# TorchIO-project/torchio

Measured on AMD Instinct MI355X. Metric: volumes/s (256^3 float32) for Compose[affine+elastic+bias+blur+noise], higher is better.
Workload: dtype f32; 1 GPU; Compose[Affine(+-10deg,0.9-1.1,+-5mm),ElasticDeformation(7^3cp,7.5mm),BiasField,Blur(0.5-2mm),Noise] on 1x256^3 f32, per-instance params; batch_per_gpu=8, global_batch=8, noise_rng=philox, resample_precision=tight, stencil_precision=fast, parallelism=batch-split x1 (no data-path collective)

## Files before the change

### include/tio_hip.h

```cpp
#ifndef TIO_HIP_H
#define TIO_HIP_H

#include <stdint.h>

#ifdef __cplusplus
extern "C" {
#endif

#define TIO_ABI_VERSION 18
#define TIO_MAX_IMAGES 8

typedef enum tio_status {
  TIO_OK = 0,
  TIO_ERR_INVALID_ARGUMENT = -1,
  TIO_ERR_UNSUPPORTED_DTYPE = -2,
  TIO_ERR_LAUNCH = -3,
  TIO_ERR_NO_DEVICE = -4,
  TIO_ERR_UNSUPPORTED_CONFIG = -5
} tio_status;

typedef enum tio_dtype {
  TIO_F32 = 0,
  TIO_F64 = 1,
  TIO_F16 = 2,
// ... 276 lines not shown

int tio_kspace_add_spikes(const void* x, void* y, int32_t dtype, int32_t batch, int32_t channels, const int32_t shape[3],
                          const int32_t* params_dev, int32_t params_words, int32_t max_count, const float* tables_dev,
                          const float* peaks_dev, const uint8_t* active_dev, void* stream);

#define TIO_MAX_SEGMENTS 32

int tio_kspace_segment_mix(const void* const* segments, int32_t n_segments, const int32_t* bounds,
                           const float* mix_dev, void* out, int32_t dtype, int32_t batch,
                           int32_t channels, const int32_t shape[3], const uint8_t* active_dev,
                           void* stream);
int tio_kspace_mix_table(int32_t length, int32_t n_segments, const int32_t* bounds, float* table_host);

#define TIO_HOST_MT_STATE_BYTES 2688
typedef struct tio_host_mt_state { uint64_t opaque[TIO_HOST_MT_STATE_BYTES / 8]; } tio_host_mt_state;
int tio_host_mt19937_seed(tio_host_mt_state* state, uint64_t seed);
int tio_host_mt19937_randn(tio_host_mt_state* state, float* out, int64_t n, int32_t n_threads);

int64_t tio_host_mt19937_plan_words(int64_t n);
int tio_host_mt19937_plan(tio_host_mt_state* state, int64_t n, uint32_t* plan_host, int64_t capacity_words, int64_t* used_words,
                          int32_t n_threads);
int64_t tio_host_mt19937_plan_begin(tio_host_mt_state* state, int64_t n, uint32_t* plan_host, int64_t capacity_words, int32_t n_threads);
int tio_host_mt19937_plan_end(int64_t handle, int64_t* used_words);
int tio_mt19937_randn_device(const uint32_t* plan_host, const uint32_t* plan_dev, float* out_dev, void* stream);
int tio_host_mt19937_plan_prefix(tio_host_mt_state* state, int64_t n, uint32_t* plan_host, int64_t capacity_words, int64_t* prefix_words,
                                 int64_t* used_words, int64_t* total_blocks);
int tio_host_mt19937_segment_polynomials(int64_t segment_blocks, int32_t count, uint32_t* out);
int tio_mt19937_device_snapshots(uint32_t* plan_dev, int64_t total_blocks, int64_t segment_blocks, const uint32_t* polys_dev, void* stream);
int tio_mt19937_add_noise_device(const uint32_t* plan_host, const uint32_t* plan_dev, const float* x_dev, float* out_dev,
                                 int64_t n_per_element, float mean, float std, const float* mean_dev, const float* std_dev,
                                 void* stream);

#define TIO_PCA_MAX_CHANNELS 1024

int64_t tio_channel_scatter_workspace_bytes(int32_t batch, int32_t channels, int64_t voxels);
int tio_channel_scatter_plan(int32_t batch, int32_t channels, int64_t voxels, int32_t out[4]);
int tio_channel_scatter(const float* x, int32_t batch, int32_t channels, int64_t voxels, double* mean, double* scatter,
                        void* workspace_dev, int64_t workspace_bytes, void* stream);

int tio_channel_project(const float* x, int32_t batch, int32_t channels, int64_t voxels, const float* center_dev,
                        const float* weights_dev, const float* offset_dev, int32_t components, int32_t clip, float* y,
                        void* stream);

#define TIO_POINTS_BLOCK_DOUBLES 40
#define TIO_POINTS_MAX_ITERATIONS 50
#define TIO_POINTS_TOLERANCE 1.0e-7
int tio_points_warp(const float* points, float* out, int8_t* status, int64_t n_total, const int32_t* offsets_host,
                    const int32_t* offsets_dev, int32_t batch, const double* blocks_dev, const float* control_points_dev,
                    int64_t control_floats, void* stream);

#define TIO_CENTRE_SEGMENT 2048
#define TIO_CENTRE_MAX_LABELS 64
typedef struct tio_centre_record {
  double total;
  int32_t invalid;
  int32_t reserved;
} tio_centre_record;
int tio_centre_law_sums(const void* weights, int32_t element_type, int32_t label_mode, const double* label_values,
                        const float* label_weights, int32_t n_labels, const int32_t shape[3], const int32_t patch[3],
                        double* prefix_dev, tio_centre_record* record_dev, void* stream);
int tio_centre_draw(const void* weights, int32_t element_type, int32_t label_mode, const double* label_values,
                    const float* label_weights, int32_t n_labels, const int32_t shape[3], const int32_t patch[3],
                    const double* prefix_dev, const tio_centre_record* record_dev, int64_t n_draws, uint64_t seed,
                    const double* uniforms_dev, double* uniforms_out_dev, int64_t* centres_dev, int32_t* corners_dev, void* stream);

int tio_patch_gather(const void* x, void* y, int32_t element_bytes, int32_t channels, const int32_t shape[3], const int32_t patch[3],
                     const int32_t* corners_dev, int32_t n_patches, void* stream);

typedef struct tio_nifti_layout {
  int32_t disk_type;
  int32_t swap_bytes;
  int32_t shape[3];
  int32_t channels;
  int32_t scaled;
  double slope, inter;
} tio_nifti_layout;
int tio_nifti_decode(const void* raw_dev, void* y, int32_t out_type, int32_t batch, const tio_nifti_layout* layout, void* stream);

int tio_abi_version(void);
const char* tio_last_error(void);
int tio_device_count(void);
void tio_reload_env(void);
int tio_launch_streams(int64_t bytes_written);

#ifdef __cplusplus
}
#endif
#endif
```

### torchio_amd/csrc/api.hip

```cpp
#include <stdarg.h>
#include <stdio.h>
#include <stdlib.h>
#include <string.h>

#include <algorithm>
#include <atomic>
#include <mutex>

#include "common.hpp"

namespace tio {

static thread_local char g_error[512] = "";

void set_error(const char* fmt, ...) {
  va_list ap;
  va_start(ap, fmt);
  vsnprintf(g_error, sizeof(g_error), fmt, ap);
  va_end(ap);
}

int fail(int status, const char* fmt, ...) {
  va_list ap;
  va_start(ap, fmt);
  vsnprintf(g_error, sizeof(g_error), fmt, ap);
  va_end(ap);
  return status;
}

int check_launch(const char* what) {
  const hipError_t err = hipGetLastError();
  if (err != hipSuccess) return fail(TIO_ERR_LAUNCH, "%s: launch failed: %s", what, hipGetErrorString(err));
  return TIO_OK;
}

static std::atomic<const EnvSwitches*> g_env{nullptr};
static std::mutex g_env_mu;

static const EnvSwitches* parse_env() {
  EnvSwitches* e = new EnvSwitches();
  auto num = [](const char* name, int unset) { const char* v = getenv(name); return v != nullptr ? atoi(v) : unset; };
  e->nearest_kernel = num("TIO_NEAREST_KERNEL", 1) != 0;
  if (const char* v = getenv("TIO_NEAREST_EPS")) { e->has_nearest_eps = 1; e->nearest_eps = static_cast<float>(atof(v)); }
  if (const char* v = getenv("TIO_RESAMPLE_PATH")) e->resample_path = strcmp(v, "gather") == 0 ? 1 : (strcmp(v, "tile") == 0 ? 2 : 0);
  e->tile_ablate = num("TIO_TILE_ABLATE", 0);
  e->resample_exact = getenv("TIO_RESAMPLE_EXACT") != nullptr;
  if (const char* v = getenv("TIO_FAST_KERNEL")) e->fast_kernel = strcmp(v, "brick") == 0 ? 1 : (strcmp(v, "planned") == 0 ? 2 : 0);
  e->planned_lean = num("TIO_PLANNED_LEAN", 1) != 0;
  e->exact_plan = num("TIO_EXACT_PLAN", -1);
  e->exact_lean = num("TIO_EXACT_LEAN", -1);
  e->lean_interleave = num("TIO_LEAN_INTERLEAVE", 1);
  e->lean_multi = num("TIO_LEAN_MULTI", 1);
  e->nearest_exact = num("TIO_NEAREST_EXACT", 1);
  e->lean_pair = num("TIO_LEAN_PAIR", 1);
  e->lean_label = num("TIO_LEAN_LABEL", 1);
  e->fast_fill_recheck = num("TIO_FAST_FILL_RECHECK", 1) != 0;
  e->conv_no_fuse = getenv("TIO_CONV_NO_FUSE") != nullptr;
  e->conv_ring = getenv("TIO_CONV_RING") != nullptr;
  if (const char* v = getenv("TIO_STREAM_BYTES")) e->stream_bytes = std::max<long long>(0, atoll(v));
  return e;
}

const EnvSwitches& env_switches() {
  const EnvSwitches* e = g_env.load(std::memory_order_acquire);
  if (e != nullptr) return *e;
  std::lock_guard<std::mutex> lock(g_env_mu);
  e = g_env.load(std::memory_order_acquire);
  if (e == nullptr) { e = parse_env(); g_env.store(e, std::memory_order_release); }
  return *e;
}

}

extern "C" void tio_reload_env(void) {
  std::lock_guard<std::mutex> lock(tio::g_env_mu);
  tio::g_env.store(tio::parse_env(), std::memory_order_release);
}

extern "C" int tio_launch_streams(int64_t bytes_written) { return tio::launch_streams(bytes_written) ? 1 : 0; }

extern "C" int tio_abi_version(void) { return TIO_ABI_VERSION; }

extern "C" const char* tio_last_error(void) { return tio::g_error; }

extern "C" int tio_device_count(void) {
  int n = 0;
  if (hipGetDeviceCount(&n) != hipSuccess) {
    (void)hipGetLastError();
    return 0;
  }
  return n;
}
```

### torchio_amd/csrc/common.hpp

```cpp
#pragma once

#include <hip/hip_runtime.h>
#include <stdint.h>

#include <type_traits>

#include "../../include/tio_hip.h"

namespace tio {

void set_error(const char* fmt, ...);
int fail(int status, const char* fmt, ...);
int check_launch(const char* what);

struct EnvSwitches {
  int nearest_kernel = 1;
  int has_nearest_eps = 0;
  float nearest_eps = 0.0f;
  int resample_path = 0;
  int tile_ablate = 0;
  int resample_exact = 0;
  int fast_kernel = 0;
  int planned_lean = 1;
  int exact_plan = -1;
  int exact_lean = -1;
  int nearest_exact = 1;
  int lean_pair = 1;
  int lean_label = 1;
  int lean_multi = 1;
  int lean_interleave = 1;
  int fast_fill_recheck = 1;
  int conv_no_fuse = 0;
  int conv_ring = 0;
  int64_t stream_bytes = -1;
};
const EnvSwitches& env_switches();

constexpr int64_t kStreamBytes = 256ll << 20;
inline bool launch_streams(int64_t bytes_written) {
  const int64_t threshold = env_switches().stream_bytes;
  return bytes_written > (threshold >= 0 ? threshold : kStreamBytes);
}

__device__ __forceinline__ float bf16_bits_to_float(uint16_t h) {
  return __uint_as_float(static_cast<uint32_t>(h) << 16);
}

__device__ __forceinline__ uint16_t float_to_bf16_bits(float f) {
  uint32_t x = __float_as_uint(f);
  if ((x & 0x7FFFFFFFu) > 0x7F800000u) return 0x7FC0u;
  x += 0x7FFFu + ((x >> 16) & 1u);
  return static_cast<uint16_t>(x >> 16);
}

template <int DT>
struct Elem;
template <>
struct Elem<TIO_F32> {
  using type = float;
  static __device__ __forceinline__ float load(const void* p, int64_t i) { return static_cast<const float*>(p)[i]; }
  static __device__ __forceinline__ void store(void* p, int64_t i, float v) { static_cast<float*>(p)[i] = v; }
};
template <>
struct Elem<TIO_F64> {
  using type = double;
  static __device__ __forceinline__ float load(const void* p, int64_t i) {
    return static_cast<float>(static_cast<const double*>(p)[i]);
  }
  static __device__ __forceinline__ void store(void* p, int64_t i, float v) {
    static_cast<double*>(p)[i] = static_cast<double>(v);
  }
};
template <>
struct Elem<TIO_F16> {
  using type = _Float16;
  static __device__ __forceinline__ float load(const void* p, int64_t i) {
    return static_cast<float>(static_cast<const _Float16*>(p)[i]);
  }
  static __device__ __forceinline__ void store(void* p, int64_t i, float v) {
    asm volatile("" : "+v"(v));
    static_cast<_Float16*>(p)[i] = static_cast<_Float16>(v);
  }
};
template <>
struct Elem<TIO_BF16> {
  using type = uint16_t;
  static __device__ __forceinline__ float load(const void* p, int64_t i) {
    return bf16_bits_to_float(static_cast<const uint16_t*>(p)[i]);
  }
  static __device__ __forceinline__ void store(void* p, int64_t i, float v) {
    static_cast<uint16_t*>(p)[i] = float_to_bf16_bits(v);
  }
};
#define TIO_INT_ELEM(CODE, T)                                                                  \
  template <>                                                                                  \
  struct Elem<CODE> {                                                                          \
    using type = T;                                                                            \
    static __device__ __forceinline__ float load(const void* p, int64_t i) {                   \
      return static_cast<float>(static_cast<const T*>(p)[i]);                                  \
    }                                                                                          \
    static __device__ __forceinline__ void store(void* p, int64_t i, float v) {                \
      static_cast<T*>(p)[i] = static_cast<T>(static_cast<int64_t>(v));     \
    }                                                                                          \
  };
TIO_INT_ELEM(TIO_U8, uint8_t)
TIO_INT_ELEM(TIO_I8, int8_t)
TIO_INT_ELEM(TIO_I16, int16_t)
TIO_INT_ELEM(TIO_I32, int32_t)
TIO_INT_ELEM(TIO_I64, int64_t)
#undef TIO_INT_ELEM

__device__ __forceinline__ float load_as_float(const void* p, int dtype, int64_t i) {
  switch (dtype) {
    case TIO_F32: return Elem<TIO_F32>::load(p, i);
    case TIO_F64: return Elem<TIO_F64>::load(p, i);
    case TIO_F16: return Elem<TIO_F16>::load(p, i);
// ... 154 lines not shown
```

### torchio_amd/csrc/resample.hip

```cpp
#include <type_traits>
#include <stdlib.h>
#include <string.h>

#include <mutex>
#include <vector>
#include <algorithm>

#include "resample_args.hpp"
#include "resample_coords.hpp"

namespace tio {

constexpr int kTileI = 8;
constexpr int kRowsPerBlock = 4;
constexpr int kLanes = 64;
constexpr int kMaxCpLds = 6144;
constexpr int kLdsFloatsPerCU = 40960;
constexpr int kPlannedMinBricks = 12288;
constexpr int kTileMinCap = 6144;
constexpr int kTileBlocksPerCU = 3;

template <int DT>
__device__ __forceinline__ void sample_interior(const ImgArgs& g, int b, int64_t n_in, int64_t n_out, int64_t o_idx,
                                                const float (&w)[8], int base, int dJK, int dK, int offn) {
// ... 425 lines not shown
#define TIO_CALL(DT) sample_boundary<DT>(g, b, n_in, n_out, o_idx, w, off, okbits, mask, offn, okn)
        TIO_DISPATCH_IMAGE(DTMODE, g.dtype, TIO_CALL)
#undef TIO_CALL
      }
    }
  }
}

}

#include "resample_exact_chain.hpp"
#include "resample_tile.hpp"
#include "resample_line.hpp"
#include "resample_plan.hpp"
#include "resample_fast.hpp"
#include "resample_lean_exact.hpp"
#include "resample_nearest.hpp"

namespace {
struct PlanSlot {
  int device;
  hipStream_t stream;
  int* ptr = nullptr;
  size_t cap = 0;
  std::mutex busy;
};
struct PlanLease {
  std::unique_lock<std::mutex> hold;
  int* ptr = nullptr;
};
}

static PlanLease plan_workspace(hipStream_t s, size_t bytes) {
  static std::mutex registry_mu;
  static std::vector<PlanSlot*> registry;
  PlanLease lease;
  int device = 0;
  if (hipGetDevice(&device) != hipSuccess) return lease;
  PlanSlot* slot = nullptr;
  {
    std::lock_guard<std::mutex> lock(registry_mu);
    for (PlanSlot* sl : registry)
      if (sl->device == device && sl->stream == s) slot = sl;
    if (slot == nullptr) {
      slot = new PlanSlot();
      slot->device = device; slot->stream = s;
      registry.push_back(slot);
    }
  }
  lease.hold = std::unique_lock<std::mutex>(slot->busy);
  if (slot->cap < bytes) {
    if (slot->ptr != nullptr) {
      (void)hipStreamSynchronize(s);
      (void)hipFree(slot->ptr);
      slot->ptr = nullptr; slot->cap = 0;
    }
    if (hipMalloc(&slot->ptr, bytes) != hipSuccess) { slot->ptr = nullptr; return lease; }
    if (hipMemsetAsync(slot->ptr, 0, tio::kPlanHeaderInts * sizeof(int), s) != hipSuccess) { (void)hipFree(slot->ptr); slot->ptr = nullptr; return lease; }
    slot->cap = bytes;
  }
  lease.ptr = slot->ptr;
  return lease;
}

namespace {
using namespace tio;

using RowsKernel = void (*)(ResampleArgs);
using BrickKernel = void (*)(ResampleArgs, const int*);
using LeanKernel = void (*)(LeanArgs);

unsigned magic_u32(unsigned n) { return n > 1 ? 0xFFFFFFFFu / n + 1u : 0u; }

template <typename Args>
int set_tiles(Args& a, int ti, int tj, int tk, unsigned* blocks) {
  a.tiles_k = (a.Ko + tk - 1) / tk; a.tiles_j = (a.Jo + tj - 1) / tj; a.tiles_i = (a.Io + ti - 1) / ti;
  a.magic_k = magic_u32(a.tiles_k); a.magic_j = magic_u32(a.tiles_j); a.magic_i = magic_u32(a.tiles_i);
  const int64_t n = static_cast<int64_t>(a.B) * a.tiles_i * a.tiles_j * a.tiles_k;
  if (n >= (1LL << 31)) return fail(TIO_ERR_INVALID_ARGUMENT, "tio_resample3d: grid too large");
  *blocks = static_cast<unsigned>(n);
  return TIO_OK;
}

template <typename Kernel>
int reserve_lds(Kernel kernel, size_t bytes) {
  if (bytes > 48 * 1024 && hipFuncSetAttribute(reinterpret_cast<const void*>(kernel), hipFuncAttributeMaxDynamicSharedMemorySize, static_cast<int>(bytes)) != hipSuccess)
    return fail(TIO_ERR_LAUNCH, "tio_resample3d: cannot reserve %zu bytes of LDS", bytes);
  return TIO_OK;
}

int control_floats(const ResampleArgs& a) { return a.cp != nullptr ? a.ni * a.nj * a.nk * 3 : 0; }
bool control_points_fit_lds(const ResampleArgs& a) { return control_floats(a) > 0 && control_floats(a) <= kMaxCpLds; }

struct Plan {
  PlanLease lease;
  int* ptr = nullptr;
  bool made_ahead = false;
};
int acquire_plan(const tio_resample_geom* geom, size_t need, hipStream_t s, Plan* plan) {
  if (geom->plan_dev != nullptr && geom->plan_bytes >= static_cast<int64_t>(need) && (reinterpret_cast<uintptr_t>(geom->plan_dev) & 15) == 0) {
    plan->ptr = static_cast<int*>(const_cast<void*>(geom->plan_dev)) + kPlanHeaderInts;
    plan->made_ahead = true;
    return TIO_OK;
  }
  plan->lease = plan_workspace(s, need);
  if (plan->lease.ptr == nullptr) return fail(TIO_ERR_LAUNCH, "tio_resample3d: cannot allocate the brick plan");
  plan->ptr = plan->lease.ptr + kPlanHeaderInts;
  return TIO_OK;
}

void enqueue_planner(const ResampleArgs& a, int* plan, int n_items, hipStream_t s) {
  const int plan_lanes = plan_group(a.cp != nullptr);
  const int plan_threads = n_items * plan_lanes > a.B ? n_items * plan_lanes : a.B;
  const dim3 plan_grid((plan_threads + 255) / 256);
  with_bools([&](auto elastic) { hipLaunchKernelGGL((plan_bricks_kernel<elastic.value, 16, 16, 16>), plan_grid, dim3(256), 0, s, a, plan, n_items); }, a.cp != nullptr);
}

int plan_bricks(const tio_resample_geom* geom, ResampleArgs& a, size_t plan_need, hipStream_t s, Plan* plan, int* n_items) {
  unsigned bricks = 0;
  if (const int st = set_tiles(a, 16, 16, 16, &bricks)) return st;
  *n_items = static_cast<int>(bricks);
  if (const int st = acquire_plan(geom, plan_need, s, plan)) return st;
  if (!plan->made_ahead) enqueue_planner(a, plan->ptr, *n_items, s);
  return TIO_OK;
}

struct FoldedMin {
  uint32_t* keys = nullptr;
  MinOuts outs{};
  int channels = 0;
};
int take_folded_min(ResampleArgs& a, bool allowed, hipStream_t s, FoldedMin* m) {
  for (int i = 0; i < a.n_images; i++) m->channels += a.img[i].out_min != nullptr ? a.img[i].channels : 0;
  if (m->channels == 0 || m->channels > kMinChannels || !allowed) {
    m->channels = 0;
    for (int i = 0; i < a.n_images; i++) a.img[i].out_min = nullptr;
    return TIO_OK;
  }
  int cap = 0;
  m->keys = min_workspace(s, m->channels * kMinSlots, &cap, 1);
  if (m->keys == nullptr) return fail(TIO_ERR_LAUNCH, "tio_resample3d: cannot allocate the reduction workspace");
  int slot = 0;
  for (int i = 0; i < a.n_images; i++)
    if (a.img[i].out_min != nullptr) {
      a.img[i].min_keys = m->keys + slot * kMinSlots;
      for (int c = 0; c < a.img[i].channels; c++) m->outs.p[slot + c] = a.img[i].out_min + c;
      slot += a.img[i].channels;
    }
  return TIO_OK;
}

void finish_folded_min(const FoldedMin& m, hipStream_t s) {
  if (m.channels > 0)
    hipLaunchKernelGGL(min_finish_kernel, dim3(static_cast<unsigned>(m.channels)), dim3(kMinSlots), 0, s, m.keys, m.outs, m.channels);
}

int check_geometry(const tio_resample_geom* geom, ResampleArgs& a) {
  if (geom->batch < 0) return fail(TIO_ERR_INVALID_ARGUMENT, "tio_resample3d: negative batch");
  if (geom->batch == 0) return TIO_OK;
  if (geom->mapping_dev == nullptr) return fail(TIO_ERR_INVALID_ARGUMENT, "tio_resample3d: mapping_dev is null");
  for (int d = 0; d < 3; d++) {
    if (geom->in_shape[d] < 1 || geom->out_shape[d] < 1)
      return fail(TIO_ERR_INVALID_ARGUMENT, "tio_resample3d: shapes must be >= 1");
  }
  const int64_t n_in = static_cast<int64_t>(geom->in_shape[0]) * geom->in_shape[1] * geom->in_shape[2];
  const int64_t n_out = static_cast<int64_t>(geom->out_shape[0]) * geom->out_shape[1] * geom->out_shape[2];
  if (n_in >= (1LL << 31) || n_out >= (1LL << 31))
    return fail(TIO_ERR_INVALID_ARGUMENT, "tio_resample3d: more than 2^31 voxels per channel");
  if (geom->passthrough_dev != nullptr && n_in != n_out)
    return fail(TIO_ERR_INVALID_ARGUMENT, "tio_resample3d: passthrough needs in_shape == out_shape");
  if (geom->control_points_dev != nullptr) {
    for (int d = 0; d < 3; d++)
      if (geom->cp_shape[d] < 1) return fail(TIO_ERR_INVALID_ARGUMENT, "tio_resample3d: bad cp_shape");
  }

  a.B = geom->batch;
  a.I = geom->in_shape[0]; a.J = geom->in_shape[1]; a.K = geom->in_shape[2];
  a.Io = geom->out_shape[0]; a.Jo = geom->out_shape[1]; a.Ko = geom->out_shape[2];
  a.affine_first = geom->affine_first;
  a.mapping = geom->mapping_dev;
  a.mapping_batched = geom->mapping_batched;
  a.cp = geom->control_points_dev;
  a.cp_batched = geom->cp_batched;
  a.ni = geom->cp_shape[0]; a.nj = geom->cp_shape[1]; a.nk = geom->cp_shape[2];
  a.cp_skip = geom->cp_skip_dev;
  a.passthrough = geom->passthrough_dev;
  const float* sp = geom->affine_first ? geom->in_spacing : geom->out_spacing;
  a.unit_spacing = 1;
  a.short_div = 1;
  for (int d = 0; d < 3; d++) {
    a.sp[d] = sp[d];
    a.rsp[d] = 1.0f / sp[d];
    if (sp[d] != 1.0f) a.unit_spacing = 0;
    const int size = geom->in_shape[d];
// ... 336 lines not shown
    if (const int st = reserve_lds(kernel_label_one, r.lds)) return st;
    la.lab_in = nn.img[0].in; la.lab_out = nn.img[0].out; la.lab_es = label->es;
  }
  int launches_left = channels;
  bool have_first = false;
  for (int i = 0; i < a.n_images; i++) {
    const ImgArgs& g = a.img[i];
    for (int c = 0; c < g.channels; c++) {
      --launches_left;
      if (pairs && !have_first && launches_left > 0) {
        set_lean_channel<false>(la, g, c);
        have_first = true;
        continue;
      }
      la.last_use = !plan.made_ahead && launches_left == 0;
      la.min_keys = (fold && g.min_keys != nullptr) ? g.min_keys + c * kMinSlots : nullptr;
      const bool with_label = label_here && launches_left == 0;
      if (have_first) set_lean_channel<true>(la, g, c);
      else set_lean_channel<false>(la, g, c);
      const LeanKernel launch = have_first ? (with_label ? kernel_label_pair : kernel_pair) : (with_label ? kernel_label_one : kernel);
      have_first = false;
      hipLaunchKernelGGL(launch, grid, block, r.lds, s, la);
      if (kernel_multi != nullptr) hipLaunchKernelGGL(kernel_multi, grid_multi, block, r.lds, s, la);
    }
  }
  finish_folded_min(fm, s);
  if (label_here) label->es = 0;
  return check_launch("tio_resample3d");
}

int resample3d_impl(const tio_resample_geom* geom, int32_t n_images, const tio_resample_image* images, void* stream, bool* folded) {
  *folded = false;
  if (geom == nullptr || images == nullptr) return fail(TIO_ERR_INVALID_ARGUMENT, "tio_resample3d: null argument");
  if (n_images < 1 || n_images > TIO_MAX_IMAGES)
    return fail(TIO_ERR_INVALID_ARGUMENT, "tio_resample3d: n_images=%d not in [1, %d]", n_images, TIO_MAX_IMAGES);
  ResampleArgs a{};
  int status = check_geometry(geom, a);
  if (status != TIO_OK || a.B == 0) return status;
  ResampleArgs pv = a, spl = a;
  pv.any_linear = 1;
  NearestArgs nn = make_nearest_args(a);
  FloatGroup group;
  const EnvSwitches& env = env_switches();
  if ((status = sort_images(n_images, images, env, a, pv, spl, nn, group)) != TIO_OK) return status;

  hipStream_t s = static_cast<hipStream_t>(stream);
  LabelRide label;
  if (nn.n_images > 0) {
    const bool floats_alone = a.n_images > 0 && pv.n_images == 0 && spl.n_images == 0 && !group.any_adjoint;
    if ((status = launch_nearest(nn, a.short_div != 0, floats_alone, env, s, &label)) != TIO_OK) return status;
    if (a.n_images == 0 && pv.n_images == 0 && spl.n_images == 0) return check_launch("tio_resample3d");
  }
  if (pv.n_images > 0) {
    if ((status = launch_label_pv(pv, s)) != TIO_OK) return status;
    if (a.n_images == 0 && spl.n_images == 0) return check_launch("tio_resample3d");
  }
  if (spl.n_images > 0) {
    if ((status = launch_bspline(spl, s)) != TIO_OK) return status;
    if (a.n_images == 0) return check_launch("tio_resample3d");
  }

  const FloatRoad road = choose_float_road(*geom, a, group, env);
  apply_road(a, road);
  switch (road.kind) {
    case kRoadGather: status = launch_gather(a, group.dtmode, s); break;
    case kRoadBrick: case kRoadPlannedBrick: case kRoadFastBrick: status = launch_brick(geom, a, road, group.dtmode, s); break;
    case kRoadPlannedFast: status = launch_planned_fast(geom, a, road, pv.n_images == 0, s, folded); break;
    case kRoadPlannedLean: case kRoadLeanExact: status = launch_lean(geom, a, road, pv.n_images == 0, nn, &label, s, folded); break;
  }
  if (label.es != 0) launch_nearest_exact(nn, label.es, label.blocks, label.lds, s);
  return status;
}

int choose_plan_road(const tio_resample_geom* geom, ResampleArgs* a, FloatRoad* road) {
  const int status = check_geometry(geom, *a);
  if (status != TIO_OK) return status;
  a->any_linear = 1;
  *road = choose_float_road(*geom, *a, FloatGroup{}, env_switches());
  return TIO_OK;
}

}

extern "C" int64_t tio_resample3d_plan_bytes(const tio_resample_geom* geom) {
  if (geom == nullptr || geom->batch < 1) return 0;
  ResampleArgs a{};
  FloatRoad road;
  return choose_plan_road(geom, &a, &road) == TIO_OK ? static_cast<int64_t>(road.plan_need) : 0;
}

extern "C" int tio_resample3d_plan(const tio_resample_geom* geom, void* plan_dev, int64_t plan_bytes, void* stream) {
  if (geom == nullptr || geom->batch < 1) return tio::fail(TIO_ERR_INVALID_ARGUMENT, "tio_resample3d_plan: no geometry / empty batch");
  ResampleArgs a{};
  FloatRoad road;
  if (const int st = choose_plan_road(geom, &a, &road)) return st;
  if (road.plan_need == 0) return tio::fail(TIO_ERR_INVALID_ARGUMENT, "tio_resample3d_plan: this geometry's launch does not start from a plan");
  if (plan_dev == nullptr || plan_bytes < static_cast<int64_t>(road.plan_need) || (reinterpret_cast<uintptr_t>(plan_dev) & 15) != 0)
    return tio::fail(TIO_ERR_INVALID_ARGUMENT, "tio_resample3d_plan: the plan needs %zu bytes, 16-byte aligned", road.plan_need);
  apply_road(a, road);
  unsigned bricks = 0;
  if (const int st = set_tiles(a, 16, 16, 16, &bricks)) return st;
  hipStream_t s = static_cast<hipStream_t>(stream);
  if (a.plan_multi && hipMemsetAsync(plan_dev, 0, kPlanHeaderInts * sizeof(int), s) != hipSuccess)
    return tio::fail(TIO_ERR_LAUNCH, "tio_resample3d_plan: cannot reset the brick plan");
  enqueue_planner(a, static_cast<int*>(plan_dev) + kPlanHeaderInts, static_cast<int>(bricks), s);
  return tio::check_launch("tio_resample3d_plan");
}

extern "C" int tio_resample3d(const tio_resample_geom* geom, int32_t n_images, const tio_resample_image* images, void* stream) {
  bool folded = false;
  const int status = resample3d_impl(geom, n_images, images, stream, &folded);
  if (status != TIO_OK || folded || geom == nullptr || images == nullptr || geom->batch < 1) return status;
  const int64_t n_out = static_cast<int64_t>(geom->out_shape[0]) * geom->out_shape[1] * geom->out_shape[2];
  for (int i = 0; i < n_images; i++) {
    const tio_resample_image& im = images[i];
    if (im.out_min_dev == nullptr || im.interp == TIO_LINEAR_ADJOINT) continue;
    const int st = tio_channel_min(im.out, im.dtype, im.channels, n_out, im.out_min_dev, stream);
    if (st != TIO_OK) return st;
  }
  return TIO_OK;
}
```

### torchio_amd/csrc/resample_args.hpp

```cpp
#pragma once
#include "common.hpp"

namespace tio {
struct ImgArgs {
  const void* in;
  void* out;
  const float* fill;
  int channels;
  int dtype;
  int interp;
  const double* labels;
  int n_labels;
  double pad_label;
  float* out_min;
  uint32_t* min_keys;
};

struct ResampleArgs {
  int B;
  int I, J, K;
  int Io, Jo, Ko;
  int affine_first;
  const float* mapping;
  int mapping_batched;
  const float* cp;
  int cp_batched;
  int ni, nj, nk;
  const uint8_t* cp_skip;
  const uint8_t* passthrough;
  float sp[3], rsp[3];
  int unit_spacing;
  float scale_i, scale_j, scale_k;
  float den[3], rden[3];
  float size_m1[3];
  float dh[3], rdh[3], half_h[3];
  int short_div;
  int any_linear, any_nearest;
  int n_images;
  ImgArgs img[TIO_MAX_IMAGES];
  int tiles_k, tiles_j, tiles_i;
  unsigned magic_k, magic_j, magic_i;
  int cp_lds;
  int tile_cap;
  int any_fill;
  int plan_multi;
  int fill_recheck;
};
}
```

### torchio_amd/csrc/resample_plan.hpp

```cpp
#pragma once
#include "resample_args.hpp"
#include "resample_tile.hpp"
#include "resample_line.hpp"

namespace tio {

struct StreamBox {
  int kind, bx0, by0, za, Lx, Ly, cpr, interior;
};

struct StageLanes {
  int cpr;
  int rpi;
  int row_l, gz_rel;
  unsigned goff;
  bool lane_ok;
};

__device__ __forceinline__ void stage_lanes(StageLanes& sl, int cpr, int K, int lane) {
  if (cpr == sl.cpr) return;
  const float rcp = __builtin_amdgcn_rcpf(static_cast<float>(cpr));
  sl.cpr = cpr;
  sl.row_l = static_cast<int>((static_cast<float>(lane) + 0.5f) * rcp);
  const int ch_l = lane - sl.row_l * cpr;
  sl.rpi = __builtin_amdgcn_readfirstlane(static_cast<int>(64.0f * rcp + 1e-3f));
  sl.lane_ok = sl.row_l < sl.rpi;
  sl.gz_rel = 4 * ch_l;
  sl.goff = static_cast<unsigned>(sl.row_l * K + 4 * ch_l) * 4u;
}

template <int NW, int AUX = 0>
__device__ __forceinline__ int stream_stage_packed(float* __restrict__ tile, const float* __restrict__ src, const StreamBox& bx, int I, int J,
                                                    int K, int wave, int lane, StageLanes& sl, int skip_mod = 0) {
  typedef __attribute__((address_space(1))) const char* global_byte_ptr;
  stage_lanes(sl, bx.cpr, K, lane);
  const int rpi = sl.rpi;
  const int total_rows = bx.Lx * bx.Ly;
  const int n_instr = __builtin_amdgcn_readfirstlane(static_cast<int>((static_cast<float>(total_rows + rpi - 1) + 0.5f) * __builtin_amdgcn_rcpf(static_cast<float>(rpi))));
  const int step = NW * rpi;
  const float rcp_ly = __builtin_amdgcn_rcpf(static_cast<float>(bx.Ly));
  const int step_p = __builtin_amdgcn_readfirstlane(static_cast<int>((static_cast<float>(step) + 0.5f) * rcp_ly));
  const int step_r = step - step_p * bx.Ly;
  int row = wave * rpi + sl.row_l;
  int p = static_cast<int>((static_cast<float>(row) + 0.5f) * rcp_ly);
  int r = row - p * bx.Ly;
  const unsigned plane_b = static_cast<unsigned>(J) * static_cast<unsigned>(K) * 4u, row_b = static_cast<unsigned>(K) * 4u;
  unsigned off = static_cast<unsigned>(p) * plane_b + static_cast<unsigned>(r) * row_b + static_cast<unsigned>(sl.gz_rel) * 4u;
  const unsigned step_b = static_cast<unsigned>(step_p) * plane_b + static_cast<unsigned>(step_r) * row_b;
  const unsigned wrap_b = plane_b - static_cast<unsigned>(bx.Ly) * row_b;
  global_byte_ptr origin = (global_byte_ptr)(src) + ((static_cast<int64_t>(bx.bx0) * J + bx.by0) * K + bx.za) * 4;
  const int dgroup = rpi * bx.cpr * 4;
  float* lp = tile + wave * dgroup;
  int issued = 0;
  const bool ch_ok = static_cast<unsigned>(bx.za + sl.gz_rel) < static_cast<unsigned>(K);
  int it = 0;
  for (int n = wave; n < n_instr; n += NW, it++) {
    const bool in_box = sl.lane_ok & (row < total_rows) & !(skip_mod > 0 && (it % skip_mod) == skip_mod - 1);
    if (bx.interior) {
      if (in_box) __builtin_amdgcn_global_load_lds(origin + off, (fast_lds_wptr)(lp), 16, 0, AUX);
      issued++;
    } else {
      const bool in_vol = in_box & ch_ok & (static_cast<unsigned>(bx.bx0 + p) < static_cast<unsigned>(I)) &
                          (static_cast<unsigned>(bx.by0 + r) < static_cast<unsigned>(J));
      if (__builtin_amdgcn_ballot_w64(in_vol) != 0ull) issued++;
      if (in_vol) __builtin_amdgcn_global_load_lds(origin + off, (fast_lds_wptr)(lp), 16, 0, AUX);
      else if (in_box) lds_zero_chunk(lp + 4 * lane);
    }
    row += step; p += step_p; r += step_r; off += step_b;
    if (r >= bx.Ly) { r -= bx.Ly; p += 1; off += wrap_b; }
    lp += NW * dgroup;
  }
  return issued;
}

struct PipePlan {
  int b, it, jt, kt;
  int i_begin, j_lo, k_lo, i_count, nv, nw;
  int fast;
  StreamBox bx;
};

template <int TI, int TJ, int TK>
__device__ __forceinline__ void pipe_decode(const ResampleArgs& a, unsigned tile, PipePlan& p) {
  const unsigned t1 = fastdiv_exact(tile, a.magic_k, a.tiles_k);
  p.kt = tile - t1 * a.tiles_k;
  const unsigned t2 = fastdiv_exact(t1, a.magic_j, a.tiles_j);
  p.jt = t1 - t2 * a.tiles_j;
  const unsigned t3 = fastdiv_exact(t2, a.magic_i, a.tiles_i);
  p.it = t2 - t3 * a.tiles_i;
  p.b = static_cast<int>(t3);
  p.i_begin = p.it * TI; p.j_lo = p.jt * TJ; p.k_lo = p.kt * TK;
  p.i_count = min(TI, a.Io - p.i_begin); p.nv = min(TJ, a.Jo - p.j_lo); p.nw = min(TK, a.Ko - p.k_lo);
  p.fast = 0;
}

__device__ __forceinline__ void pipe_brick_frame(FastFrameG& f, int j_lo, int k_lo) {
#pragma unroll
  for (int r = 0; r < 3; r++)
    f.c[r] = static_cast<double>(f.m[4 * r + 1]) * j_lo + static_cast<double>(f.m[4 * r + 2]) * k_lo + static_cast<double>(f.m[4 * r + 3]);
  f.j_lo = j_lo; f.k_lo = k_lo;
}

__device__ __forceinline__ void pipe_vertex(const ResampleArgs& a, const FastFrameG& f, int vtx, int u0, int n, int nv, int nw, int (&r)[6], bool& bad) {
  const int u_lo = u0, u_hi = u0 + n - 1;
  int du, dv, dw;
  if (f.elastic) { du = vtx % 3; dv = (vtx / 3) % 3; dw = vtx / 9; } else { du = vtx & 1; dv = (vtx >> 1) & 1; dw = vtx >> 2; }
  bool dense = false;
  float u = du == 0 ? static_cast<float>(u_lo) : static_cast<float>(u_hi);
  float v = dv == 0 ? 0.0f : static_cast<float>(nv - 1);
  float w = dw == 0 ? 0.0f : static_cast<float>(nw - 1);
  if (f.elastic) {
    if (du == 2) u = fast_breakpoint(f.sci, f.ni, u_lo, u_hi, dense);
    if (dv == 2) v = fast_breakpoint(f.scj, f.nj, f.j_lo, f.j_lo + nv - 1, dense) - static_cast<float>(f.j_lo);
    if (dw == 2) w = fast_breakpoint(f.sck, f.nk, f.k_lo, f.k_lo + nw - 1, dense) - static_cast<float>(f.k_lo);
  }
  float x, y, z;
  fast_coord(f, u, v, w, x, y, z);
  constexpr float kMargin = 1.0f / 64.0f;
  bad = !(fabsf(x) <= 1e30f) | !(fabsf(y) <= 1e30f) | !(fabsf(z) <= 1e30f) | dense;
  const float capx = a.size_m1[0] + 1.0f + kTileFar, capy = a.size_m1[1] + 1.0f + kTileFar, capz = a.size_m1[2] + 1.0f + kTileFar;
  r[0] = -static_cast<int>(fminf(fmaxf(floorf(x - kMargin), -kTileFar), capx));
  r[1] = static_cast<int>(fminf(fmaxf(floorf(x + kMargin), -kTileFar), capx));
  r[2] = -static_cast<int>(fminf(fmaxf(floorf(y - kMargin), -kTileFar), capy));
  r[3] = static_cast<int>(fminf(fmaxf(floorf(y + kMargin), -kTileFar), capy));
  r[4] = -static_cast<int>(fminf(fmaxf(floorf(z - kMargin), -kTileFar), capz));
  r[5] = static_cast<int>(fminf(fmaxf(floorf(z + kMargin), -kTileFar), capz));
}

enum : int { kPlanHeaderInts = 16, kDescMulti = 4, kPassInts = 8, kPassesPerBrick = 4, kPassStaged = 0, kPassOutside = 1, kPassSlow = 2 };

struct PlanBox {
  int xmin, ymin, za, Lx, Ly, cpr, interior, outside, fits;
};
__device__ __forceinline__ PlanBox plan_box(const ResampleArgs& a, const int (&ext)[7], bool weird) {
  PlanBox pb;
  const int xmin = -ext[0], xmax = ext[1], ymin = -ext[2], ymax = ext[3], zmin = -ext[4], zmax = ext[5];
  const bool wrd = weird | (ext[6] != 0);
  pb.interior = (xmin >= 0) & (xmax + 1 <= a.I - 1) & (ymin >= 0) & (ymax + 1 <= a.J - 1) & (zmin >= 0) & (zmax + 1 <= a.K - 1) & !wrd;
  pb.outside = ((xmax + 1 < 0) | (xmin > a.I - 1) | (ymax + 1 < 0) | (ymin > a.J - 1) | (zmax + 1 < 0) | (zmin > a.K - 1)) & !wrd;
  pb.za = zmin & ~3; pb.Lx = xmax + 2 - xmin; pb.Ly = ymax + 2 - ymin;
  const int Lz = ((zmax + 1 + 4) & ~3) - pb.za;
  pb.fits = !wrd && (Lz <= 256) && (pb.Lx <= 4096) && (pb.Ly <= 4096) && (static_cast<int64_t>(pb.Lx) * pb.Ly * Lz <= static_cast<int64_t>(a.tile_cap));
  pb.xmin = xmin; pb.ymin = ymin; pb.cpr = Lz >> 2;
  return pb;
}
__device__ __forceinline__ PlanBox plan_pass_box(const ResampleArgs& a, const int (&ext)[7], bool weird) {
  PlanBox pb = plan_box(a, ext, weird);
  if (pb.fits && !box_address_fits(pb.xmin, pb.ymin, pb.za, pb.Lx, pb.Ly, pb.cpr)) pb.fits = 0;
  return pb;
}
constexpr int plan_group(bool elastic_possible) { return elastic_possible ? 32 : 8; }

template <bool ELASTIC_POSSIBLE, int TI, int TJ, int TK>
__global__ __launch_bounds__(256) void plan_bricks_kernel(const ResampleArgs a, int* __restrict__ plan, int n_items) {
  constexpr int GROUP = plan_group(ELASTIC_POSSIBLE);
  const int gtid = blockIdx.x * blockDim.x + threadIdx.x;
  const float ratio[3] = {a.half_h[0] / a.dh[0], a.half_h[1] / a.dh[1], a.half_h[2] / a.dh[2]};
  if (gtid < a.B) {
    const float* m = a.mapping + (a.mapping_batched ? gtid * 12 : 0);
    float* fr = reinterpret_cast<float*>(plan) + gtid * 16;
    for (int q = 0; q < 12; q++) fr[q] = m[q] * ratio[q >> 2];
    {
      float mm[12];
      for (int q = 0; q < 12; q++) mm[q] = m[q];
      fr[12] = fast_fill_margin(mm, static_cast<float>(a.Io), static_cast<float>(a.Jo), static_cast<float>(a.Ko), a.size_m1[0] + 1.0f,
                                a.size_m1[1] + 1.0f, a.size_m1[2] + 1.0f);
    }
    fr[13] = __int_as_float(a.tile_cap);
    for (int q = 14; q < 16; q++) fr[q] = 0.0f;
  }
  const int t = gtid / GROUP, v = gtid % GROUP;
  if (t >= n_items) return;
  PipePlan p;
// ... 145 lines not shown
```

### torchio_amd/csrc/resample_tile.hpp

```cpp
#pragma once
#include "resample_args.hpp"
#include "resample_coords.hpp"

namespace tio {

#define TIO_OPAQUE3(A, B, C, DEP) asm("" : "+v"(A), "+v"(B), "+v"(C) : "s"(DEP))

constexpr int kTileRedInts = 512;
constexpr int kTileBoxBase = 448;
constexpr int kTileStashPlanes = 4;
#ifndef TILE_GROUP
#define TILE_GROUP 4
#endif

__device__ __forceinline__ unsigned fastdiv(unsigned n, unsigned magic, unsigned d) {
  return d == 1 ? n : __umulhi(n, magic);
}
__device__ __forceinline__ unsigned fastdiv_magic(unsigned d) { return d > 1 ? 0xFFFFFFFFu / d + 1u : 0u; }
__device__ __forceinline__ unsigned fastdiv_exact(unsigned n, unsigned magic, unsigned d) {
  if (d == 1) return n;
  unsigned q = __umulhi(n, magic);
  if (q * d > n) q--;
  return q;
}
// ... 369 lines not shown
  const bool vec_ok = (g.dtype == TIO_F32) & ((a.K & 3) == 0) & ((reinterpret_cast<uintptr_t>(g.in) & 15) == 0);
  TileAddr ta;
  ta.ox = static_cast<float>(bx.bx0); ta.oy = static_cast<float>(bx.by0); ta.oz = static_cast<float>(bx.za);
  ta.sYb = bx.Lz * 4; ta.sXb = bx.Ly * bx.Lz * 4; ta.sXYb = ta.sXb + ta.sYb;
  ta.sYbf = static_cast<float>(ta.sYb); ta.sXbf = static_cast<float>(ta.sXb);
  ta.base_f = static_cast<float>(tile_lds_addr);
  const int es = dtype_size(g.dtype);
  const int64_t bc = static_cast<int64_t>(b) * g.channels + c;
  if (!prestaged) __syncthreads();
  if (prestaged) {
    tile_dma_wait();
  } else if (vec_ok) {
    stage_brick_dma<NT>(s_tile, static_cast<const float*>(g.in) + bc * n_in, tid, bx, a.I, a.J, a.K);
    tile_dma_wait();
  } else {
    stage_brick_generic<NT, DTMODE>(s_tile, static_cast<const char*>(g.in) + bc * n_in * es, g.dtype, tid, bx, a.I, a.J, a.K);
  }
  __syncthreads();
  const bool has_fill = g.fill != nullptr;
  typedef __attribute__((address_space(4))) const float* const_float_ptr;
  const float fillv = has_fill ? ((const_float_ptr)g.fill)[c] : 0.0f;
  const int64_t slab_b = static_cast<int64_t>(slab) * es;
  char* out_c = static_cast<char*>(g.out) + (bc * n_out + static_cast<int64_t>(i_begin) * slab) * es;
  const unsigned urow = static_cast<unsigned>(row) * static_cast<unsigned>(es);
#pragma unroll
  for (int q = 0; q < NQ; q++) {
    if (q < q_begin || q >= q_end) continue;
    char* out_t = out_c + (q * QT) * slab_b;
    if (bx.interior && full) {
      constexpr int G = TILE_GROUP < QT ? TILE_GROUP : QT;
#pragma unroll
      for (int u0 = 0; u0 < QT; u0 += G) {
        TapSet ts[G];
#pragma unroll
        for (int u = 0; u < G; u++) tile_issue_interior<LAUNDER>(ts[u], X[q * QT + u0 + u], Y[q * QT + u0 + u], Z[q * QT + u0 + u], ta, c);
        __builtin_amdgcn_sched_barrier(0);
#pragma unroll
        for (int u = 0; u < G; u++) {
          store_at<DTMODE>(out_t, g.dtype, urow, FAST ? tile_finish_fast(ts[u]) : tile_finish(ts[u]));
          out_t += slab_b;
        }
        __builtin_amdgcn_sched_barrier(0);
      }
    } else if (bx.interior) {
#pragma unroll
      for (int u = 0; u < QT; u++) {
        const int t = q * QT + u;
        TapSet ts;
        tile_issue_interior<LAUNDER>(ts, X[t], Y[t], Z[t], ta, c);
        const float val = FAST ? tile_finish_fast(ts) : tile_finish(ts);
        if (col_active && t < i_count) store_at<DTMODE>(out_t, g.dtype, urow, val);
        out_t += slab_b;
        __builtin_amdgcn_sched_barrier(0);
      }
    } else {
#pragma unroll
      for (int u = 0; u < QT; u++) {
        const int t = q * QT + u;
        TapSet ts;
        float x = X[t], y = Y[t], z = Z[t];
        if constexpr (LAUNDER) TIO_OPAQUE3(x, y, z, c);
        tile_issue_interior<false>(ts, x, y, z, ta, c);
        float val = FAST ? tile_finish_fast(ts) : tile_finish(ts);
        if (has_fill) val = (tile_mask(ts, x, y, z, hx, hy, hz) > 0.5f) ? val : fillv;
        if (full || (col_active && t < i_count)) store_at<DTMODE>(out_t, g.dtype, urow, val);
        out_t += slab_b;
        if ((u & 1) == 1) __builtin_amdgcn_sched_barrier(0);
      }
    }
  }
}

template <bool ELASTIC_POSSIBLE, int DTMODE, int TI, int TJ, int TK, int OCC, bool FAST = false>
__global__ __launch_bounds__(TJ* TK, (TJ * TK) / 256 * OCC) void resample_tile_kernel(const ResampleArgs a, const int* __restrict__ plan) {
  constexpr int NT = TJ * TK, NW = NT / 64;
  constexpr int NQ = 4, QT = TI / NQ;
  static_assert(TI % NQ == 0 && QT <= kTileStashPlanes, "unsupported brick depth");
  extern __shared__ __attribute__((aligned(16))) float smem[];
  float* s_cp = smem;
  int* s_red = reinterpret_cast<int*>(smem + a.cp_lds);
  float* s_tile = smem + a.cp_lds + kTileRedInts;

  const unsigned tile = xcd_remap(blockIdx.x, gridDim.x);
  const unsigned t1 = fastdiv_exact(tile, a.magic_k, a.tiles_k);
  const int kt = tile - t1 * a.tiles_k;
  const unsigned t2 = fastdiv_exact(t1, a.magic_j, a.tiles_j);
  const int jt = t1 - t2 * a.tiles_j;
  const unsigned t3 = fastdiv_exact(t2, a.magic_i, a.tiles_i);
  const int it = t2 - t3 * a.tiles_i;
  const int b = t3;

  const int tid = threadIdx.x;
  const int lane = tid & 63;
  const int wave = __builtin_amdgcn_readfirstlane(tid >> 6);
  const int tk = tid % TK, tj = tid / TK;
  const int jo_raw = jt * TJ + tj, ko_raw = kt * TK + tk;
  const bool col_active = (jo_raw < a.Jo) & (ko_raw < a.Ko);
  const int jo = min(jo_raw, a.Jo - 1), ko = min(ko_raw, a.Ko - 1);
  const int i_begin = it * TI;
  const int i_count = min(TI, a.Io - i_begin);
  const int i_last = i_begin + i_count - 1;
  const bool full = (i_count == TI) & ((jt + 1) * TJ <= a.Jo) & ((kt + 1) * TK <= a.Ko);

  const int64_t n_in = static_cast<int64_t>(a.I) * a.J * a.K;
  const int64_t n_out = static_cast<int64_t>(a.Io) * a.Jo * a.Ko;
  const int row = jo * a.Ko + ko;
  const int slab = a.Jo * a.Ko;

  if (a.passthrough != nullptr && a.passthrough[b] != 0) {
    if (col_active) {
      for (int t = 0; t < i_count; t++) {
        const int64_t o_idx = static_cast<int64_t>(i_begin + t) * slab + row;
        for (int im = 0; im < a.n_images; im++) {
          const ImgArgs& g = a.img[im];
          const int es = dtype_size(g.dtype);
          for (int c = 0; c < g.channels; c++) {
            const int64_t off = (static_cast<int64_t>(b) * g.channels + c) * n_out + o_idx;
            const char* s = static_cast<const char*>(g.in) + off * es;
            char* d = static_cast<char*>(g.out) + off * es;
            for (int e = 0; e < es; e++) d[e] = s[e];
          }
        }
      }
    }
    return;
  }

  const float* m = a.mapping + (a.mapping_batched ? b * 12 : 0);
  const float m00 = m[0], m01 = m[1], m02 = m[2], m03 = m[3];
  const float m10 = m[4], m11 = m[5], m12 = m[6], m13 = m[7];
  const float m20 = m[8], m21 = m[9], m22 = m[10], m23 = m[11];
  bool weird = false;
#pragma unroll
  for (int q = 0; q < 12; q++) weird |= (__float_as_uint(m[q]) & 0x7FFFFFFFu) > 0x7149F2CAu;

  bool elastic = false, plane_cached = false;
  const float* cp = nullptr;
  int cp_bad = 0;
  int ia = 0, ib = 0;
  Lerp1D li_lane = {0, 0, 0.0f, 0.0f};
  if constexpr (ELASTIC_POSSIBLE) {
    elastic = !(a.cp_skip != nullptr && a.cp_skip[b] != 0);
    if (elastic) {
      const int n_cp = a.ni * a.nj * a.nk * 3;
      const float* cp_global = a.cp + (a.cp_batched ? static_cast<int64_t>(b) * n_cp : 0);
      cp = cp_global;
      li_lane = lerp_index(min(i_begin + (lane & (TI - 1)), i_last), a.ni, a.Io, a.scale_i);
      ia = __builtin_amdgcn_readlane(li_lane.i0, 0);
      ib = __builtin_amdgcn_readlane(li_lane.i1, TI - 1);
      plane_cached = ib - ia <= 2;
    }
    if (elastic && !plane_cached) {
      const int n_cp = a.ni * a.nj * a.nk * 3;
      const float* cp_global = cp;
      int bad = 0;
      if (a.cp_lds > 0) {
        for (int t = tid; t < n_cp; t += NT) {
          const float v = cp_global[t];
          bad |= !(fabsf(v) <= 1e30f);
          s_cp[t] = v;
        }
        cp = s_cp;
      } else {
        for (int t = tid; t < n_cp; t += NT) bad |= !(fabsf(cp_global[t]) <= 1e30f);
      }
      weird |= (__syncthreads_or(bad) != 0);
    }
  }

  float X[TI], Y[TI], Z[TI];
  float lo[3], hi[3];
  const float cj = static_cast<float>(jo), ck = static_cast<float>(ko);
  const float hx = a.size_m1[0], hy = a.size_m1[1], hz = a.size_m1[2];
// ... 318 lines not shown
```

Before: 6322 volumes/s.

## Add slab-ordered brick traversal for resample tiles via planner descriptors

```diff
diff --git a/include/tio_hip.h b/include/tio_hip.h
--- a/include/tio_hip.h
+++ b/include/tio_hip.h
@@ -382,6 +382,8 @@
 int tio_device_count(void);
 void tio_reload_env(void);
 int tio_launch_streams(int64_t bytes_written);
+int tio_brick_order(const int32_t tiles[3], int32_t slab, int64_t item, int32_t out[3]);
+int tio_brick_slab(const int32_t tiles[3]);
 
 #ifdef __cplusplus
 }
diff --git a/torchio_amd/csrc/api.hip b/torchio_amd/csrc/api.hip
--- a/torchio_amd/csrc/api.hip
+++ b/torchio_amd/csrc/api.hip
@@ -57,6 +57,7 @@
   e->fast_fill_recheck = num("TIO_FAST_FILL_RECHECK", 1) != 0;
   e->conv_no_fuse = getenv("TIO_CONV_NO_FUSE") != nullptr;
   e->conv_ring = getenv("TIO_CONV_RING") != nullptr;
+  e->brick_slab = std::max(0, num("TIO_BRICK_SLAB", 0));
   if (const char* v = getenv("TIO_STREAM_BYTES")) e->stream_bytes = std::max<long long>(0, atoll(v));
   return e;
 }
diff --git a/torchio_amd/csrc/common.hpp b/torchio_amd/csrc/common.hpp
--- a/torchio_amd/csrc/common.hpp
+++ b/torchio_amd/csrc/common.hpp
@@ -32,6 +32,7 @@
   int fast_fill_recheck = 1;
   int conv_no_fuse = 0;
   int conv_ring = 0;
+  int brick_slab = 0;
   int64_t stream_bytes = -1;
 };
 const EnvSwitches& env_switches();
diff --git a/torchio_amd/csrc/resample.hip b/torchio_amd/csrc/resample.hip
--- a/torchio_amd/csrc/resample.hip
+++ b/torchio_amd/csrc/resample.hip
@@ -531,6 +531,8 @@
   return TIO_OK;
 }
 
+int choose_brick_slab(int tiles_i, const EnvSwitches& env) { return std::min(std::max(env.brick_slab, 1), std::max(tiles_i, 1)); }
+
 template <typename Kernel>
 int reserve_lds(Kernel kernel, size_t bytes) {
   if (bytes > 48 * 1024 && hipFuncSetAttribute(reinterpret_cast<const void*>(kernel), hipFuncAttributeMaxDynamicSharedMemorySize, static_cast<int>(bytes)) != hipSuccess)
@@ -558,7 +560,8 @@
   return TIO_OK;
 }
 
-void enqueue_planner(const ResampleArgs& a, int* plan, int n_items, hipStream_t s) {
+void enqueue_planner(ResampleArgs& a, int* plan, int n_items, hipStream_t s) {
+  a.brick_slab = choose_brick_slab(a.tiles_i, env_switches());
   const int plan_lanes = plan_group(a.cp != nullptr);
   const int plan_threads = n_items * plan_lanes > a.B ? n_items * plan_lanes : a.B;
   const dim3 plan_grid((plan_threads + 255) / 256);
@@ -1061,6 +1064,23 @@
 
 }
 
+extern "C" int tio_brick_order(const int32_t tiles[3], int32_t slab, int64_t item, int32_t out[3]) {
+  if (tiles == nullptr || out == nullptr) return tio::fail(TIO_ERR_INVALID_ARGUMENT, "tio_brick_order: null argument");
+  if (tiles[0] < 1 || tiles[1] < 1 || tiles[2] < 1 || static_cast<int64_t>(tiles[0]) * tiles[1] * tiles[2] >= (1LL << 31))
+    return tio::fail(TIO_ERR_INVALID_ARGUMENT, "tio_brick_order: bad tile counts");
+  if (slab < 1) return tio::fail(TIO_ERR_INVALID_ARGUMENT, "tio_brick_order: slab %d is below 1", slab);
+  if (item < 0 || item >= static_cast<int64_t>(tiles[0]) * tiles[1] * tiles[2])
+    return tio::fail(TIO_ERR_INVALID_ARGUMENT, "tio_brick_order: item %lld is not a brick of %d x %d x %d", static_cast<long long>(item), tiles[0], tiles[1], tiles[2]);
+  const tio::BrickPos p = tio::brick_order(tiles[0], tiles[1], tiles[2], slab, static_cast<unsigned>(item));
+  out[0] = p.it; out[1] = p.jt; out[2] = p.kt;
+  return TIO_OK;
+}
+
+extern "C" int tio_brick_slab(const int32_t tiles[3]) {
+  if (tiles == nullptr || tiles[0] < 1 || tiles[1] < 1 || tiles[2] < 1) return tio::fail(TIO_ERR_INVALID_ARGUMENT, "tio_brick_slab: bad tile counts");
+  return choose_brick_slab(tiles[0], tio::env_switches());
+}
+
 extern "C" int64_t tio_resample3d_plan_bytes(const tio_resample_geom* geom) {
   if (geom == nullptr || geom->batch < 1) return 0;
   ResampleArgs a{};
diff --git a/torchio_amd/csrc/resample_args.hpp b/torchio_amd/csrc/resample_args.hpp
--- a/torchio_amd/csrc/resample_args.hpp
+++ b/torchio_amd/csrc/resample_args.hpp
@@ -45,5 +45,6 @@
   int any_fill;
   int plan_multi;
   int fill_recheck;
+  int brick_slab;
 };
 }
diff --git a/torchio_amd/csrc/resample_order.hpp b/torchio_amd/csrc/resample_order.hpp
--- /dev/null
+++ b/torchio_amd/csrc/resample_order.hpp
@@ -0,0 +1,28 @@
+#pragma once
+#include "common.hpp"
+
+namespace tio {
+
+struct BrickPos {
+  int it, jt, kt;
+};
+
+__host__ __device__ inline BrickPos brick_order(unsigned tiles_i, unsigned tiles_j, unsigned tiles_k, unsigned slab, unsigned item) {
+  const unsigned T = slab < 1u ? 1u : (slab > tiles_i ? tiles_i : slab);
+  const unsigned slab_items = T * tiles_j * tiles_k;
+  const unsigned i_hi = item / slab_items;
+  const unsigned r = item - i_hi * slab_items;
+  const unsigned left = tiles_i - i_hi * T;
+  const unsigned depth = left < T ? left : T;
+  const unsigned row = depth * tiles_k;
+  const unsigned jt = r / row;
+  const unsigned r2 = r - jt * row;
+  const unsigned i_lo = r2 / tiles_k;
+  BrickPos p;
+  p.it = static_cast<int>(i_hi * T + i_lo);
+  p.jt = static_cast<int>(jt);
+  p.kt = static_cast<int>(r2 - i_lo * tiles_k);
+  return p;
+}
+
+}
diff --git a/torchio_amd/csrc/resample_plan.hpp b/torchio_amd/csrc/resample_plan.hpp
--- a/torchio_amd/csrc/resample_plan.hpp
+++ b/torchio_amd/csrc/resample_plan.hpp
@@ -2,6 +2,7 @@
 #include "resample_args.hpp"
 #include "resample_tile.hpp"
 #include "resample_line.hpp"
+#include "resample_order.hpp"
 
 namespace tio {
 
@@ -82,13 +83,11 @@
 
 template <int TI, int TJ, int TK>
 __device__ __forceinline__ void pipe_decode(const ResampleArgs& a, unsigned tile, PipePlan& p) {
-  const unsigned t1 = fastdiv_exact(tile, a.magic_k, a.tiles_k);
-  p.kt = tile - t1 * a.tiles_k;
-  const unsigned t2 = fastdiv_exact(t1, a.magic_j, a.tiles_j);
-  p.jt = t1 - t2 * a.tiles_j;
-  const unsigned t3 = fastdiv_exact(t2, a.magic_i, a.tiles_i);
-  p.it = t2 - t3 * a.tiles_i;
-  p.b = static_cast<int>(t3);
+  const unsigned bpe = static_cast<unsigned>(a.tiles_i) * a.tiles_j * a.tiles_k;
+  const unsigned b = tile / bpe;
+  const BrickPos pos = brick_order(a.tiles_i, a.tiles_j, a.tiles_k, a.brick_slab, tile - b * bpe);
+  p.it = pos.it; p.jt = pos.jt; p.kt = pos.kt;
+  p.b = static_cast<int>(b);
   p.i_begin = p.it * TI; p.j_lo = p.jt * TJ; p.k_lo = p.kt * TK;
   p.i_count = min(TI, a.Io - p.i_begin); p.nv = min(TJ, a.Jo - p.j_lo); p.nw = min(TK, a.Ko - p.k_lo);
   p.fast = 0;
diff --git a/torchio_amd/csrc/resample_tile.hpp b/torchio_amd/csrc/resample_tile.hpp
--- a/torchio_amd/csrc/resample_tile.hpp
+++ b/torchio_amd/csrc/resample_tile.hpp
@@ -475,13 +475,20 @@
   float* s_tile = smem + a.cp_lds + kTileRedInts;
 
   const unsigned tile = xcd_remap(blockIdx.x, gridDim.x);
-  const unsigned t1 = fastdiv_exact(tile, a.magic_k, a.tiles_k);
-  const int kt = tile - t1 * a.tiles_k;
-  const unsigned t2 = fastdiv_exact(t1, a.magic_j, a.tiles_j);
-  const int jt = t1 - t2 * a.tiles_j;
-  const unsigned t3 = fastdiv_exact(t2, a.magic_i, a.tiles_i);
-  const int it = t2 - t3 * a.tiles_i;
-  const int b = t3;
+  int kt, jt, it, b;
+  if (plan != nullptr) {
+    typedef __attribute__((address_space(4))) const int* const_int_ptr;
+    const_int_ptr d = (const_int_ptr)(plan + a.B * 16) + static_cast<size_t>(tile) * kDescInts;
+    b = d[10]; it = d[11] / TI; jt = d[12] / TJ; kt = d[13] / TK;
+  } else {
+    const unsigned t1 = fastdiv_exact(tile, a.magic_k, a.tiles_k);
+    kt = tile - t1 * a.tiles_k;
+    const unsigned t2 = fastdiv_exact(t1, a.magic_j, a.tiles_j);
+    jt = t1 - t2 * a.tiles_j;
+    const unsigned t3 = fastdiv_exact(t2, a.magic_i, a.tiles_i);
+    it = t2 - t3 * a.tiles_i;
+    b = t3;
+  }
 
   const int tid = threadIdx.x;
   const int lane = tid & 63;
```

Result: no change. 6321 volumes/s, median of 2 (-0.0%).
